# medical-genomics-group/sgVAMP-py

Hardware: AMD Instinct MI355X
Metric: VAMP iterations/sec (and effective LD-matvec GB/s) at M markers, K cohorts (higher is better)
Workload: dtype f64

## Files before the change

sgvamp-py_amd/csrc/common.h:

```cpp
#pragma once
#include <hip/hip_runtime.h>
#include <cstdint>

namespace sgv {

constexpr int WAVE = 64;
constexpr int VTHREADS = 256;
constexpr int CHUNK = 1024;
constexpr int PADV = 128;
constexpr int MAXC = 16;
constexpr int MAXK = 32;
constexpr int MAXCOH = 1024;
constexpr int MAXKG = 8;
constexpr int MAXL = 8;

typedef double d2 __attribute__((ext_vector_type(2)));

#define SGV_GLOBAL __attribute__((address_space(1)))
template <class T>
__device__ __forceinline__ T ldg(const T* p) {
  return *(const SGV_GLOBAL T*)p;
}
template <class T>
__device__ __forceinline__ T ldg_nt(const T* p) {
// ... 234 lines not shown
        if (pa.dot[c]) acc = pre.dot[b] * o;
      }
      const double sm = wave_sum(acc);
      if (lane == 0) s_w[wid][c] = sm;
    }
    __syncthreads();
  }
  if (threadIdx.x < NC)
    partials[(int64_t)pn.part * NC + t] = ((s_w[0][t] + s_w[1][t]) + s_w[2][t]) + s_w[3][t];
}

const char* ab_env(const char* name);

hipError_t launch_read_probe(const double* buf, size_t bytes, double* out, hipStream_t st);

hipError_t launch_coupling(int nc, const CouplingTask* d_tasks, int ntasks, const PassArgs& pa,
                           const double* halo, int64_t hstride, double* cpbuf, int ncp_slots,
                           hipStream_t st);
hipError_t launch_halo_pack(const PassArgs& pa, int nc, int64_t src0, int len0, int64_t src1,
                            int len1, int64_t hstride, double* send, hipStream_t st);
hipError_t launch_ld_pass(int nc, const BlkDesc* d_blks, const RowGroup* d_rg, int nrg,
                          const PassArgs& pa, double* d_partials, hipStream_t st);
int ld_pass_rows_per_group();
hipError_t launch_sym_pass(int nc, int cls, const SymItem* d_items, int nitems,
                           const PassArgs& pa, double* rowpart, double* colpart, hipStream_t st);
hipError_t launch_pk(const PassArgs& pa, int nc, int64_t mpad, double* d_pk, hipStream_t st,
                     bool paired = false);
bool strip_pk_paired(int nc);
hipError_t launch_sym_mfma(int nc, const SymStrip* d_strips, int nstrips, const SymItem* d_sitems,
                           const PassArgs& pa, const double* d_pk, double* rowpart,
                           double* colpart, bool ragged, int pair, int bits, hipStream_t st);
hipError_t launch_sym_mfma_wide(int nc, const SymStrip* d_strips, int nstrips,
                                const SymItem* d_sitems, const PassArgs& pa, const double* d_pk,
                                double* rowpart, double* colpart, bool idle_exit, hipStream_t st);
hipError_t launch_sym_finalize_wide(int nc, const SymPanelW* d_panels, int npanels,
                                    const PassArgs& pa, const double* rowpart,
                                    const double* colpart, double* partials, hipStream_t st);
hipError_t launch_band_walk(int nc, const SymWalk* d_walks, int nwalks, const SymPanel* d_panels,
                            const SymItem* d_items, const double* d_pk, int64_t pk_rows,
                            const PassArgs& pa, double* headbuf, double* carrybuf,
                            const WalkFin* d_fins, int nfins,
                            double* partials, int bits, hipStream_t st);
hipError_t launch_sym_finalize_strip(int nc, const SymPanel* d_panels, int npanels,
                                     const PassArgs& pa, const double* rowpart,
                                     const double* colpart, double* partials, bool ragged,
                                     hipStream_t st);
hipError_t launch_sym_finalize(int nc, int cls, const SymPanel* d_panels, int npanels,
                               const PassArgs& pa, const double* rowpart, const double* colpart,
                               double* partials, hipStream_t st);

hipError_t launch_reduce_blocks(const double* d_part, int nv, const int* d_begin, int nblk,
                                double* d_bsum, hipStream_t st, int op = 0, int ostride = 0,
                                int ooff = 0);
hipError_t launch_reduce_local(const double* d_part, int nv, const int* d_begin, int nblk,
                               const Map16& map, double* d_dst, hipStream_t st, int op = 0);
hipError_t launch_reduce_total(const double* d_bsum_all, int nranks, int nbmax, int nv,
                               const int* d_counts, const Map16& map, double* d_dst,
                               hipStream_t st, int op = 0);

struct DenoiseArgs {
  const double* r1[MAXK];
  double* xhat1;
  double ag[MAXK];
  double a[MAXK], gam1[MAXK];
  double sum_ag;
  double lam;
  int K, nslab;
// ... 245 lines not shown
```

sgvamp-py_amd/csrc/ldplan.hip:

```cpp
#include "ctx.h"

void free_plan(LdPlan& p){
  if (p.d_rg) (void)hipFree(p.d_rg);
  if (p.d_pbeg) (void)hipFree(p.d_pbeg);
  for (int k = 0; k < 4; ++k) {
    if (p.d_items[k]) (void)hipFree(p.d_items[k]);
    if (p.d_panels[k]) (void)hipFree(p.d_panels[k]);
  }
  for (StripSet* q : {&p.s512, &p.wide, &p.rest}) {
    if (q->d_strips) (void)hipFree(q->d_strips);
    if (q->d_sitems) (void)hipFree(q->d_sitems);
    if (q->d_panels) (void)hipFree(q->d_panels);
    if (q->d_wpanels) (void)hipFree(q->d_wpanels);
  }
  if (p.d_ctasks) (void)hipFree(p.d_ctasks);
  if (p.d_walks) (void)hipFree(p.d_walks);
  if (p.d_wpanels) (void)hipFree(p.d_wpanels);
  if (p.d_witems) (void)hipFree(p.d_witems);
  if (p.d_wfins) (void)hipFree(p.d_wfins);
  p = LdPlan();
}

void free_block(LdBlock& lb){
  if (lb.ptr) (void)hipFree(lb.ptr);
// ... 249 lines not shown
  out->ngrp = ngrp;
  out->nstrips = (int)strips.size();
  out->nsitems = (int)sitems.size();
  out->npanels = (int)sp.size();
  out->ragged = false;
  for (const SymStrip& st : strips)
    for (int i = 0; i < st.npan; ++i) out->ragged |= sitems[st.it0 + i].nc < st.ncmax;
  out->pair = (wide || out->ragged) ? 0 : mfma_pair_choice(strips, sitems);
  CHK(upload_table(c, strips, &out->d_strips));
  CHK(upload_table(c, sitems, &out->d_sitems));
  if (wide) {
    CHK(upload_table(c, sp, &out->d_wpanels));
  } else {
    std::vector<SymPanel> p512(sp.size());
    for (size_t i = 0; i < sp.size(); ++i) {
      p512[i] = sp[i].p;
      p512[i].own_sb = sp[i].sb[0];
      p512[i].own_se = sp[i].se[0];
      p512[i].oth_sb = sp[i].sb[1];
      p512[i].oth_se = sp[i].se[1];
    }
    CHK(upload_table(c, p512, &out->d_panels));
  }
  return SGV_OK;
}

static bool wide_pass(int nc) {
  if (nc < 3 || nc > 8) return false;
  const char* e = ab_env("SGV_MF_WIDE");
  if (e && (e[0] == '0' || e[0] == '1')) return e[0] == '1';
  const char* p = ab_env("SGV_MF_PAIR");
  if (p && (p[0] == '0' || p[0] == '1')) return false;
  return true;
}

constexpr int WALK_F32_MIN_NC = 3;
static bool f32_walk_on() {
  const char* e = ab_env("SGV_F32_WALK");
  return e && e[0] == '1';
}
static int band_walk_max_nc() {
  const char* e = ab_env("SGV_BAND_WALK");
  return (e && e[0] == '0') ? 0 : 8;
}

static int plan_walks(sgv_ctx* c, int ld, const std::vector<SymItem>& items,
                      const std::vector<SymPanel>& panels, LdPlan* pl) {
  if (band_walk_max_nc() == 0) return SGV_OK;
  bool any = false;
  for (int b = 0; b < c->nblk; ++b) {
    const LdBlock& lb = c->ldb[ld][b];
    if (lb.fmt != 1) continue;
    if (lb.ext <= 0 || lb.ext > (int64_t)WALK_RMAX * SYM_H) return SGV_OK;
    if (c->bn[b] + SYM_H >= ((int64_t)1 << 31) / (8 * 8)) return SGV_OK;
    any = true;
  }
  if (!any) return SGV_OK;
  if (pl->bits == 32)
    for (const SymItem& it : items)
      if (((uintptr_t)it.P + sizeof(float) * (size_t)(it.c0 - it.r0)) % 16 != 0 || it.w % 4 != 0)
        return fail(c, SGV_ERR_STATE,
                    "walk plan: f32 item (r0 %d, c0 %d, row stride %lld) is not 16-byte aligned",
                    it.r0, it.c0, (long long)it.w);
  std::vector<SymWalk> walks;
  std::vector<WalkFin> fins;
  int hs = 0, cs = 0, bp0 = 0;
// ... 306 lines not shown
    e0 = c->evpool.back();
    c->evpool.pop_back();
    e1 = c->evpool.back();
    c->evpool.pop_back();
  }
  HIPCHK(hipEventRecord(e0, c->st));
  if (pl.halo || pl.nctasks) CHK(coupling_pass(c, pl, nc, pa));
  if (pl.nrg) HIPCHK(launch_ld_pass(nc, c->d_blks[ld], pl.d_rg, pl.nrg, pa, c->d_part, c->st));
  if (pl.npanels) {
    const bool f32 = pl.bits == 32;
    const bool mf = f32 || (c->mfma_min > 0 && nc >= c->mfma_min);
    const int cls = mf ? 1 : sym_class(nc);
    if (mf) {
      const bool walk = pl.nwalks && nc <= band_walk_max_nc() &&
                        (!f32 || (nc >= WALK_F32_MIN_NC && f32_walk_on()));
      double mf_aux = 0.0;
      HIPCHK(launch_pk(pa, nc, c->Mpad, c->d_pk, c->st,
                       walk ? nc > 4 : strip_pk_paired(nc)));
      if (walk) {
        HIPCHK(launch_band_walk(nc, pl.d_walks, pl.nwalks, pl.d_wpanels, pl.d_witems, c->d_pk,
                                c->Mpad, pa,
                                c->d_whead, c->d_wcarry, pl.d_wfins, pl.nwfins, c->d_part, pl.bits,
                                c->st));
      } else {
        const bool usew = !f32 && pl.wide.nstrips > 0 && wide_pass(nc);
        bool side = false;
        auto run_set = [&](const StripSet& ss, bool wide, double* rp, double* cp) -> int {
          for (int g = 0; g < ss.ngrp; ++g) {
            const int s0 = ss.gs[g], ns = ss.gs[g + 1] - s0;
            const int p0 = ss.gp[g], npn = ss.gp[g + 1] - p0;
            const bool split = ss.ngrp > 1;
            if (wide)
              HIPCHK(launch_sym_mfma_wide(nc, ss.d_strips + s0, ns, ss.d_sitems, pa, c->d_pk, rp,
                                          cp, pl.wide_idle, c->st));
            else
              HIPCHK(launch_sym_mfma(nc, ss.d_strips + s0, ns, ss.d_sitems, pa, c->d_pk, rp, cp,
                                     ss.ragged, f32 ? 0 : ss.pair, pl.bits, c->st));
            hipStream_t fs = c->st;
            if (split) {
              HIPCHK(hipEventRecord(c->ev_grp[g % MAXGRP], c->st));
              HIPCHK(hipStreamWaitEvent(c->st_fin, c->ev_grp[g % MAXGRP], 0));
              fs = c->st_fin;
              side = true;
            }
            if (wide)
              HIPCHK(launch_sym_finalize_wide(nc, ss.d_wpanels + p0, npn, pa, rp, cp, c->d_part,
                                              fs));
            else
              HIPCHK(launch_sym_finalize_strip(nc, ss.d_panels + p0, npn, pa, rp, cp, c->d_part,
                                               ss.ragged, fs));
          }
          return SGV_OK;
        };
        if (usew) {
          CHK(run_set(pl.wide, true, c->d_rowpart, c->d_colpart));
          if (pl.rest.nstrips)
            CHK(run_set(pl.rest, false, c->d_rowpart + (size_t)pl.wide.nslots_items * SYM_H * nc,
                        c->d_colpart + (size_t)pl.wide.nstrips * MFW_CW * nc));
          mf_aux = 2.0 * 8.0 * nc * ((double)pl.wide.nsitems * SYM_H +
                                     (double)pl.wide.nstrips * MFW_CW +
                                     (double)pl.rest.nsitems * SYM_H +
                                     (double)pl.rest.nstrips * 512);
        } else {
          CHK(run_set(pl.s512, false, c->d_rowpart, c->d_colpart));
          mf_aux = 2.0 * 8.0 * nc * ((double)pl.s512.nsitems * SYM_H +
                                     (double)pl.s512.nstrips * 512);
        }
// ... 288 lines not shown
```

sgvamp-py_amd/csrc/strip_wave.h:

```cpp
#pragma once
#include "common.h"

#include <type_traits>

namespace sgv {

__device__ __forceinline__ double mfma4(double a, double b, double c) {
  return __builtin_amdgcn_mfma_f64_4x4x4f64(a, b, c, 0, 0, 0);
}

__device__ __forceinline__ void lds_order() {
  __builtin_amdgcn_fence(__ATOMIC_ACQ_REL, "wavefront");
  __builtin_amdgcn_wave_barrier();
}

template <int ORDER>
__device__ __forceinline__ void lds_wait_ge(int* ctr, int v) {
  while (__hip_atomic_load(ctr, ORDER, __HIP_MEMORY_SCOPE_WORKGROUP) < v)
    __builtin_amdgcn_s_sleep(1);
}

typedef float f2 __attribute__((ext_vector_type(2)));
template <class T>
struct Frag;
// ... 118 lines not shown
                                                  bool more, const SymItem& nx,
                                                  uint64_t nxb) const {
    const bool same = g + 1 < ng;
    NextGroup n;
    n.b = same ? curb : nxb;
    n.w = same ? cur.w : (more ? nx.w : 0);
    n.H = same ? cur.H : (more ? nx.H : 1);
    n.nc = same ? cur.nc : nx.nc;
    n.g = same ? g + 1 : 0;
    n.r0 = same ? cur.r0 : nx.r0;
    n.z = col_zero(n.r0);
    return n;
  }

  __device__ __forceinline__ void band_zero(int nci, int t, d2* cf) const {
    const int xc = cw0 + frag_col<LF>(t, lo);
#pragma unroll
    for (int a = 0; a < 4; ++a) {
      cf[a].x = xc < nci ? cf[a].x : 0.0;
      cf[a].y = xc + 1 < nci ? cf[a].y : 0.0;
    }
  }

  __device__ __forceinline__ void tile_exchange(double* sb, const d2* cf, d2* rf) const {
    lds_order();
#pragma unroll
    for (int a = 0; a < 4; ++a)
      *(d2*)(sb + 32 * (4 * (SWZ ? a ^ (bq & 2) : a) + hi) + 2 * (lo ^ hi)) = cf[a];
    lds_order();
#pragma unroll
    for (int r = 0; r < 4; ++r) rf[r] = *(const d2*)(sb + 32 * (4 * r + n4) + 2 * (pc ^ n4));
  }

  __device__ __forceinline__ void reduce_blocks(const double (&drow)[4][NG], double* wb) const {
#pragma unroll
    for (int r = 0; r < 4; ++r)
#pragma unroll
      for (int q = 0; q < NG; ++q) {
        double v = drow[r][q];
        v = v + row_ror<12>(v);
        v = v + row_ror<8>(v);
        if (bq == 0) wb[(4 * r + hi) * RW + 4 * q + n4] = v;
      }
  }

  template <int NT, int CW>
  __device__ __forceinline__ void store_colpart(double* out, int p, int ncol,
                                                const double (&dcol)[NT][2][NG]) const {
#pragma unroll
    for (int q = 0; q < NG; ++q)
      if (4 * q + n4 < ncol) {
#pragma unroll
        for (int t = 0; t < NT; ++t)
          *(d2*)(out + 4 * q * CW + frag_col<LF>(t, p)) = d2{dcol[t][0][q], dcol[t][1][q]};
      }
  }
};

template <class SW, int PD, int NT>
struct FragRing {
  static_assert(PD >= 1 && PD <= NT && NT % PD == 0, "prefetch depth divides the steps");
  static_assert(!SW::W4 || (PD == 2 && NT % 2 == 0), "LF = 2: two super-steps");
  static constexpr int RD = SW::W4 ? NT / 2 : PD;
  typename SW::RV q[RD][4];
  d2 w[SW::W4 ? 2 : 1][4];

// ... 124 lines not shown
```

sgvamp-py_amd/csrc/sym_mfma.hip:

```cpp
#include "strip_wave.h"

namespace sgv {

#ifdef SGV_MF_TRACE
constexpr int MF_TRACE_MAX = 1 << 16;
__device__ unsigned long long g_mf_trace[3 * MF_TRACE_MAX];
#define MF_TRACE_BEGIN const unsigned long long tr_t0 = wall_clock64();
#define MF_TRACE_END                                                          \
  __syncthreads();                                                            \
  if (threadIdx.x == 0 && blockIdx.x < MF_TRACE_MAX) {                        \
    g_mf_trace[3 * blockIdx.x] = tr_t0;                                       \
    g_mf_trace[3 * blockIdx.x + 1] = wall_clock64();                          \
    g_mf_trace[3 * blockIdx.x + 2] = (unsigned long long)__smid();            \
  }
#else
#define MF_TRACE_BEGIN
#define MF_TRACE_END
#endif

constexpr int F32_FORM_DEFAULT = 2;

constexpr int MF_CW = 512;
constexpr int MF_LDP = 34;

template <int NG, int PD, bool RAG = false, bool DEF = false, bool PP = false, class T = double,
          int LF = 1>
__global__ __launch_bounds__(256, 2) void k_sym_mfma(const SymStrip* __restrict__ strips,
                                                     const SymItem* __restrict__ sitems,
                                                     const double* __restrict__ pk, int ncol,
                                                     double* __restrict__ rowpart,
                                                     double* __restrict__ colpart,
                                                     const int* __restrict__ run, int pks) {
  constexpr int NW = 4;
// ... 5 lines not shown
  __shared__ __attribute__((aligned(16))) double stg[NW][16 * 32];
  const SymStrip sp = strips[blockIdx.x];
  if (run && !ldg(run)) return;
  MF_TRACE_BEGIN
  const int lane = threadIdx.x & (WAVE - 1);
  const int wid = __builtin_amdgcn_readfirstlane(threadIdx.x / WAVE);
  SymItem cur = sitems[sp.it0];
  const int cw0 = wid * WC;
  const SW sw(lane, pk + (int64_t)cur.voff * pks, pks, cur.c0, sp.ncmax, cw0, cw0 < SYM_H);
  const int nta = min(NT, sw.steps_to(sw.ncc));
  double* sb = stg[wid];
  double brow[NT][2][NG];
  sw.load_brow(brow);
  double dcol[NT][2][NG];
  zero(dcol);

  uint64_t curb = SW::pbase(cur);
  FragRing<SW, PD, NT> ring;
  double bcn[SW::NB][NG];
  ring.prime(sw, curb, cur);
  sw.load_bcol(cur.r0, cur.H, sw.col_zero(cur.r0), 0, bcn);

#pragma unroll 1
  for (int s = 0; s < sp.npan; ++s) {
    const bool more = s + 1 < sp.npan;
    const SymItem nx = sitems[sp.it0 + (more ? s + 1 : s)];
    const uint64_t nxb = more ? SW::pbase(nx) : (uint64_t)sw.pkb;
    const int ng = (cur.H + 15) / 16;
#pragma unroll 1
    for (int g = 0; g < ng; ++g) {
      const NextGroup nxt = sw.next_group(g, ng, cur, curb, more, nx, nxb);
      double bcol[4][NG];
      sw.hand_bcol(bcn, bcol);
      double drow[4][NG];
      zero(drow);
      const bool colz = sw.col_zero(cur.r0);
      const int ntp = RAG ? min(nta, sw.steps_to(cur.nc)) : nta;
      d2 rfb[DEF ? 2 : 1][4];
#pragma unroll
      for (int t = 0; t < NT; ++t) {
        d2 cf[4];
        d2* rf = rfb[DEF ? (t & 1) : 0];
        ring.step(sw, t, g, curb, cur, nxt, bcn, cf);
        if (t >= ntp) continue;
        if (RAG && cur.nc < sw.ncc) sw.band_zero(cur.nc, t, cf);
        sw.tile_exchange(sb, cf, rf);
        __builtin_amdgcn_s_setprio(1);
        if constexpr (DEF)
          mfma_step_deferred<NG, NT>(t, t == NT - 1 || t + 1 == ntp, colz, cf, rf,
                                     rfb[(t + 1) & 1], bcol, brow, dcol[t], drow);
        else
          mfma_step<NG>(colz, cf, rf, true, bcol, brow[t], dcol[t], drow);
        __builtin_amdgcn_s_setprio(0);
      }
      sw.reduce_blocks(drow, rowbuf + (wid * SYM_H + 16 * g) * RW);
    }
    __syncthreads();
    panel_rows_out<NW, NW * 64, RW>(rowbuf, cur.H, ncol, rowpart + (int64_t)cur.item * SYM_H * ncol);
    __syncthreads();
    cur = nx;
    curb = nxb;
  }
  sw.template store_colpart<NT, MF_CW>(colpart + ((int64_t)sp.slot * ncol + sw.n4) * MF_CW + cw0,
                                       sw.pc, ncol, dcol);
  MF_TRACE_END
}
// ... 22 lines not shown
  const int seg = wid & 3;
  const int h = wid >> 2;
  SymItem cur = sitems[sp.it0];
  const int cw0 = seg * 128 + h * WC;
  const SW sw(lane, pk + (int64_t)cur.voff * pks, pks, cur.c0, sp.ncmax, cw0, seg * 128 < SYM_H);
  const int nta_seg = min(4, max(0, (sw.ncc - seg * 128 + 31) / 32));
  const int nta = min(NT, max(0, nta_seg - NT * h));
  double* sb = stg[wid];
  double brow[NT][2][NG];
  sw.load_brow(brow);
  double dcol[NT][2][NG];
  zero(dcol);

  uint64_t curb = SW::pbase(cur);
  FragRing<SW, PD, NT> ring;
  double bcn[SW::NB][NG];
  ring.prime(sw, curb, cur);
  sw.load_bcol(cur.r0, cur.H, sw.col_zero(cur.r0), 0, bcn);
  if (threadIdx.x < 4) hready[threadIdx.x] = hdone[threadIdx.x] = 0;
  __syncthreads();

  int gg = 0;
#pragma unroll 1
  for (int s = 0; s < sp.npan; ++s) {
    const bool more = s + 1 < sp.npan;
    const SymItem nx = sitems[sp.it0 + (more ? s + 1 : s)];
    const uint64_t nxb = more ? SW::pbase(nx) : (uint64_t)sw.pkb;
    const int ng = (cur.H + 15) / 16;
#pragma unroll 1
    for (int g = 0; g < ng; ++g, ++gg) {
      const NextGroup nxt = sw.next_group(g, ng, cur, curb, more, nx, nxb);
      double bcol[4][NG];
      sw.hand_bcol(bcn, bcol);
      double drow[4][NG];
      zero(drow);
      const bool colz = sw.col_zero(cur.r0);
      d2 rfs[NT][4];
#pragma unroll
      for (int t = 0; t < NT; ++t) {
        d2 cf[4];
        ring.step(sw, t, g, curb, cur, nxt, bcn, cf);
        if (t >= nta) continue;
        sw.tile_exchange(sb, cf, rfs[t]);
        __builtin_amdgcn_s_setprio(1);
        mfma_step<NG>(colz, cf, rfs[t], h == 0, bcol, brow[t], dcol[t], drow);
        __builtin_amdgcn_s_setprio(0);
      }
      double* hs = &hand[gg % HS][seg][0][0];
      if (h == 0) {
        lds_wait_ge<__ATOMIC_ACQUIRE>(&hdone[seg], gg - HS + 1);
#pragma unroll
        for (int r = 0; r < 4; ++r)
#pragma unroll
          for (int q = 0; q < NG; ++q) hs[(r * NG + q) * WAVE + lane] = drow[r][q];
        __hip_atomic_store(&hready[seg], gg + 1, __ATOMIC_RELEASE, __HIP_MEMORY_SCOPE_WORKGROUP);
      }
      if (h == 1) {
        lds_wait_ge<__ATOMIC_ACQUIRE>(&hready[seg], gg + 1);
#pragma unroll
        for (int r = 0; r < 4; ++r)
#pragma unroll
          for (int q = 0; q < NG; ++q) drow[r][q] = hs[(r * NG + q) * WAVE + lane];
        __hip_atomic_store(&hdone[seg], gg + 1, __ATOMIC_RELEASE, __HIP_MEMORY_SCOPE_WORKGROUP);
        __builtin_amdgcn_s_setprio(1);
#pragma unroll
        for (int t = 0; t < NT; ++t)
// ... 37 lines not shown
  const int cw0 = wid * WC;
  const SW sw(lane, pk + (int64_t)cur.voff * PKS, PKS, cur.c0, sp.ncmax, cw0, cw0 < SYM_H);
  const int nta = min(NT, sw.steps_to(sw.ncc));
  const int nact = idle ? min(NW, (sw.ncc + WC - 1) / WC) : NW;
  if (threadIdx.x < MFW_RD) hready[threadIdx.x] = hdone[threadIdx.x] = 0;
  __syncthreads();
  if (wid >= nact) return;
  double* sb = stg[wid];
  double brow[NT][2][NG];
  sw.load_brow(brow);
  double dcol[NT][2][NG];
  zero(dcol);

  uint64_t curb = SW::pbase(cur);
  FragRing<SW, PD, NT> ring;
  double bcn[SW::NB][NG];
  ring.prime(sw, curb, cur);
  sw.load_bcol(cur.r0, cur.H, sw.col_zero(cur.r0), 0, bcn);

  double* outp = colpart + ((int64_t)sp.slot * ncol + sw.n4) * MFW_CW + cw0 + 2 * sw.pc;
  asm volatile("" : "+v"(outp));
  int gg = 0;
#pragma unroll 1
  for (int s = 0; s < sp.npan; ++s) {
    const bool more = s + 1 < sp.npan;
    const SymItem nx = sitems[sp.it0 + (more ? s + 1 : s)];
    const uint64_t nxb = more ? SW::pbase(nx) : (uint64_t)sw.pkb;
    const int ng = (cur.H + 15) / 16;
#pragma unroll 1
    for (int g = 0; g < ng; ++g) {
      const NextGroup nxt = sw.next_group(g, ng, cur, curb, more, nx, nxb);
      double bcol[4][NG];
      sw.hand_bcol(bcn, bcol);
      double drow[4][NG];
      zero(drow);
      const bool colz = sw.col_zero(cur.r0);
      d2 rfb[2][4];
#pragma unroll
      for (int t = 0; t < NT; ++t) {
        d2 cf[4];
        ring.step(sw, t, g, curb, cur, nxt, bcn, cf);
        if (t >= nta) continue;
        sw.tile_exchange(sb, cf, rfb[t & 1]);
        __builtin_amdgcn_s_setprio(1);
        mfma_step_deferred<NG, NT>(t, t == NT - 1 || t + 1 == nta, colz, cf, rfb[t & 1],
                                   rfb[(t + 1) & 1], bcol, brow, dcol[t], drow);
        __builtin_amdgcn_s_setprio(0);
      }
      const int hs = gg % MFW_RD, gen = gg / MFW_RD;
      lds_wait_ge<__ATOMIC_RELAXED>(&hdone[hs], gen);
      sw.reduce_blocks(drow, hand[hs][wid]);
      __builtin_amdgcn_fence(__ATOMIC_RELEASE, "wavefront");
      if (lane == 0)
        __hip_atomic_fetch_add(&hready[hs], 1, __ATOMIC_RELAXED, __HIP_MEMORY_SCOPE_WORKGROUP);
      if (wid == ((g & (NW - 1)) < nact ? (g & (NW - 1)) : 0)) {
        lds_wait_ge<__ATOMIC_RELAXED>(&hready[hs], nact * (gen + 1));
        __builtin_amdgcn_fence(__ATOMIC_ACQUIRE, "wavefront");
        double* dst = rowpart + ((int64_t)cur.item * SYM_H + 16 * g) * ncol;
#pragma unroll
        for (int k = 0; k < (16 * RW + WAVE - 1) / WAVE; ++k) {
          const int e = lane + WAVE * k;
          if (e < 16 * RW) {
            const int row = e / RW, cc = e - row * RW;
            const double* rr = &hand[hs][0][0] + e;
            double v = rr[0];
#pragma unroll
            for (int w = 1; w < NW; ++w) {
              const double x = rr[w * 16 * RW];
              v += w < nact ? x : 0.0;
            }
            if (16 * g + row < cur.H && cc < ncol) dst[row * ncol + cc] = v;
          }
        }
        __builtin_amdgcn_fence(__ATOMIC_RELEASE, "wavefront");
        if (lane == 0)
          __hip_atomic_store(&hdone[hs], gen + 1, __ATOMIC_RELAXED, __HIP_MEMORY_SCOPE_WORKGROUP);
      }
      ++gg;
    }
    cur = nx;
    curb = nxb;
  }
  sw.template store_colpart<NT, MFW_CW>(outp, 0, ncol, dcol);
}

typedef double d4 __attribute__((ext_vector_type(4)));
#define MFMA16(a, b, c) __builtin_amdgcn_mfma_f64_16x16x4f64((a), (b), (c), 0, 0, 0)
template <int PD, bool RAG = false, int TB = 0, class T = double, int LF = 1>
__global__ __launch_bounds__(256, 2) void k_sym_mfma16(const SymStrip* __restrict__ strips,
                                                     const SymItem* __restrict__ sitems,
                                                     const double* __restrict__ pk, int ncol,
                                                     double* __restrict__ rowpart,
                                                     double* __restrict__ colpart,
                                                     const int* __restrict__ run) {
  constexpr int LDP = MF_LDP;
  constexpr int MF_WC = MF_CW / 4;
  constexpr int MF_NT = MF_WC / 32;
  constexpr bool W4 = LF == 2;
  static_assert(!W4 || (sizeof(T) == 4 && PD == 2 && MF_NT % 2 == 0), "LF = 2: float, two super-steps");
  typedef typename std::conditional<W4, f4, typename Frag<T>::raw>::type RV;
  constexpr int RD = W4 ? MF_NT / 2 : PD;
  __shared__ double red[2][4][256];
  __shared__ __attribute__((aligned(16))) double stg[4][16 * LDP];
  constexpr bool BL = TB > 0;
  __shared__ __attribute__((aligned(16))) double bls[BL ? 4 : 1][BL ? TB * 4 : 1][WAVE][2];
  const SymStrip sp = strips[blockIdx.x];
  if (run && !ldg(run)) return;
  const int lane = threadIdx.x & (WAVE - 1);
  const int wid = __builtin_amdgcn_readfirstlane(threadIdx.x / WAVE);
  const int lo = lane & 15, hi = lane >> 4;
  SymItem cur = sitems[sp.it0];
  const int c0 = cur.c0, ncc = sp.ncmax;
  const double* pkb = pk + (int64_t)cur.voff * 16;
  const int cw0 = wid * MF_WC;
  const bool dhalf = cw0 < SYM_H;
  const int nta = W4 ? min(MF_NT, max(0, steps_upto<LF>(ncc - cw0)))
// ... 362 lines not shown
    hipLaunchKernelGGL(k_pack<16>, pg, dim3(256), 0, st, pa, nc, mpad, d_pk);
  return hipGetLastError();
}

hipError_t launch_sym_mfma(int nc, const SymStrip* d_strips, int nstrips, const SymItem* d_sitems,
                           const PassArgs& pa, const double* d_pk, double* rowpart,
                           double* colpart, bool ragged, int pair, int bits, hipStream_t st) {
  if (nc < 1 || nc > 16) return hipErrorInvalidValue;
  if (bits != 64 && bits != 32) return hipErrorInvalidValue;
  const bool f32 = bits == 32;
  if (f32 && pair) return hipErrorInvalidValue;
  if (nstrips <= 0) return hipSuccess;
  const int pks = nc > 8 ? 16 : nc <= 4 ? 4 : 8;
  switch ((nc + 3) / 4) {
    case 1: launch_mf<1>(d_strips, nstrips, d_sitems, d_pk, nc, rowpart, colpart, pa.run, pks, ragged, pair, f32, st); break;
    case 2:
      launch_mf<2, true>(d_strips, nstrips, d_sitems, d_pk, nc, rowpart, colpart, pa.run, pks,
                         ragged, pair, f32, st);
      break;
    default:
      with_strip_inst(f32, ragged, [&](auto i) {
        typedef decltype(i) I;
        hipLaunchKernelGGL((k_sym_mfma16<2, I::rag, I::rag ? 2 : 1, typename I::elem, I::lf>),
                           dim3(nstrips), dim3(256), 0, st, d_strips, d_sitems, d_pk, nc, rowpart,
                           colpart, pa.run);
      });
      break;
  }
  return hipGetLastError();
}

hipError_t launch_sym_mfma_wide(int nc, const SymStrip* d_strips, int nstrips,
                                const SymItem* d_sitems, const PassArgs& pa, const double* d_pk,
                                double* rowpart, double* colpart, bool idle_exit, hipStream_t st) {
  if (nc < 3 || nc > 8) return hipErrorInvalidValue;
  if (nstrips <= 0) return hipSuccess;
  if (nc <= 4)
    hipLaunchKernelGGL((k_sym_mfma_wide<1, 2>), dim3(nstrips), dim3(512), 0, st, d_strips,
                       d_sitems, d_pk, nc, rowpart, colpart, pa.run, idle_exit ? 1 : 0);
  else
    hipLaunchKernelGGL((k_sym_mfma_wide<2, 2, true>), dim3(nstrips), dim3(512), 0, st, d_strips,
                       d_sitems, d_pk, nc, rowpart, colpart, pa.run, idle_exit ? 1 : 0);
  return hipGetLastError();
}

hipError_t launch_sym_finalize_wide(int nc, const SymPanelW* d_panels, int npanels,
                                    const PassArgs& pa, const double* rowpart,
                                    const double* colpart, double* partials, hipStream_t st) {
  if (npanels <= 0) return hipSuccess;
#define FINW_CASE(N)                                                                         \
  case N:                                                                                    \
    hipLaunchKernelGGL(k_sym_finalize_wide<N>, dim3(npanels), dim3(256 * FIN_Q), 0, st,      \
                       d_panels, pa, rowpart, colpart, partials);                            \
    break;
  switch (nc) {
    FINW_CASE(3) FINW_CASE(4) FINW_CASE(5) FINW_CASE(6) FINW_CASE(7) FINW_CASE(8)
    default: return hipErrorInvalidValue;
  }
#undef FINW_CASE
  return hipGetLastError();
}

#ifdef SGV_MF_TRACE
extern "C" int sgv_diag_mf_trace(unsigned long long* out, int n) {
  if (n > MF_TRACE_MAX) n = MF_TRACE_MAX;
  return hipMemcpyFromSymbol(out, HIP_SYMBOL(g_mf_trace), sizeof(unsigned long long) * 3 * n) ==
                 hipSuccess ? n : -1;
}
#endif

static int fin_form(bool ragged, int nc) {
  const char* e = ab_env("SGV_FIN_FORM");
  const int v = (e && (e[0] == '1' || e[0] == '4')) ? e[0] - '0' : 0;
  return v ? v : (ragged && nc <= 8) ? 1 : 4;
}
// ... 28 lines not shown
```

Before: 29.40.

## Add warp-specialized LDS ring loader for the wide symmetric MFMA pass

Adds a new wide symmetric-LD kernel variant in which one or more dedicated loader waves stream LD panel tiles from global memory straight into an LDS ring buffer, using global_load_lds DMA with nontemporal hints. The compute waves consume slots through ready/done flags in LDS instead of issuing their own global loads, so fetching and MFMA work can overlap. The loader variant is picked by an env-tunable code, and for more than four cohorts it defaults to one loader wave, lag 3 and ring depth 6. The existing wide kernels also now prefetch the next group's column operand early. This adds a producer/consumer protocol, more LDS use and one occupancy slot per CU, which risks stalls or synchronisation overhead.

```diff
diff --git a/sgvamp-py_amd/csrc/common.h b/sgvamp-py_amd/csrc/common.h
--- a/sgvamp-py_amd/csrc/common.h
+++ b/sgvamp-py_amd/csrc/common.h
@@ -290,7 +290,8 @@
                            double* colpart, bool ragged, int pair, int bits, hipStream_t st);
 hipError_t launch_sym_mfma_wide(int nc, const SymStrip* d_strips, int nstrips,
                                 const SymItem* d_sitems, const PassArgs& pa, const double* d_pk,
-                                double* rowpart, double* colpart, bool idle_exit, hipStream_t st);
+                                double* rowpart, double* colpart, bool idle_exit, int loader,
+                                hipStream_t st);
 hipError_t launch_sym_finalize_wide(int nc, const SymPanelW* d_panels, int npanels,
                                     const PassArgs& pa, const double* rowpart,
                                     const double* colpart, double* partials, hipStream_t st);
diff --git a/sgvamp-py_amd/csrc/ldplan.hip b/sgvamp-py_amd/csrc/ldplan.hip
--- a/sgvamp-py_amd/csrc/ldplan.hip
+++ b/sgvamp-py_amd/csrc/ldplan.hip
@@ -305,6 +305,15 @@
   const char* p = ab_env("SGV_MF_PAIR");
   if (p && (p[0] == '0' || p[0] == '1')) return false;
   return true;
+}
+
+static int wide_loader(int nc) {
+  constexpr int LOADER_DEFAULT = 136;
+  const char* e = ab_env("SGV_MF_LOADER");
+  if (e && e[0] == '0') return 0;
+  if (e && e[0] && e[1] && e[2]) return std::atoi(e);
+  if (e && e[0] == '1') return LOADER_DEFAULT;
+  return nc > 4 ? LOADER_DEFAULT : 0;
 }
 
 constexpr int WALK_F32_MIN_NC = 3;
@@ -677,7 +686,7 @@
             const bool split = ss.ngrp > 1;
             if (wide)
               HIPCHK(launch_sym_mfma_wide(nc, ss.d_strips + s0, ns, ss.d_sitems, pa, c->d_pk, rp,
-                                          cp, pl.wide_idle, c->st));
+                                          cp, pl.wide_idle, wide_loader(nc), c->st));
             else
               HIPCHK(launch_sym_mfma(nc, ss.d_strips + s0, ns, ss.d_sitems, pa, c->d_pk, rp, cp,
                                      ss.ragged, f32 ? 0 : ss.pair, pl.bits, c->st));
diff --git a/sgvamp-py_amd/csrc/strip_ring.h b/sgvamp-py_amd/csrc/strip_ring.h
--- /dev/null
+++ b/sgvamp-py_amd/csrc/strip_ring.h
@@ -0,0 +1,80 @@
+#pragma once
+
+#if defined(__HIPCC__) || defined(__CUDACC__)
+#define SGV_RING_HD __host__ __device__ __forceinline__
+#else
+#define SGV_RING_HD inline
+#endif
+
+namespace sgv {
+
+constexpr int RING_NW = 8;
+constexpr int RING_HW = 4;
+constexpr int RING_WC = 128;
+constexpr int RING_NT = 4;
+constexpr int RING_SUB = 4096;
+constexpr int RING_PIECE = 1024;
+constexpr int RING_SLOT = RING_HW * RING_SUB;
+constexpr int RING_LAGMAX = 3;
+
+SGV_RING_HD constexpr bool ring_fits(int D, int NL, int LAG) {
+  return NL >= 1 && LAG >= 1 && LAG <= RING_LAGMAX && D > NL * LAG + 2;
+}
+
+SGV_RING_HD int ring_nta(int ncc, int w) {
+  const int n = (ncc - RING_WC * w + 31) / 32;
+  return n < 0 ? 0 : n > RING_NT ? RING_NT : n;
+}
+SGV_RING_HD int ring_nact(int ncc, int idle) {
+  const int n = (ncc + RING_WC - 1) / RING_WC;
+  return idle ? (n < RING_NW ? n : RING_NW) : RING_NW;
+}
+SGV_RING_HD int ring_nfg(int ncc) { return ring_nta(ncc, 0) + ring_nta(ncc, RING_HW); }
+SGV_RING_HD int ring_nwh(int ncc, int t, int h) {
+  int n = 0;
+  for (int w = RING_HW * h; w < RING_HW * h + RING_HW; ++w) n += ring_nta(ncc, w) > t ? 1 : 0;
+  return n;
+}
+SGV_RING_HD int ring_fill_q(int ncc, int t, int h) {
+  const int n4 = ring_nta(ncc, RING_HW);
+  return t + (t < n4 ? t : n4) + h;
+}
+SGV_RING_HD void ring_fill_th(int ncc, int q, int* t, int* h) {
+  const int n4 = ring_nta(ncc, RING_HW);
+  if (q < 2 * n4) {
+    *t = q >> 1;
+    *h = q & 1;
+  } else {
+    *t = q - n4;
+    *h = 0;
+  }
+}
+SGV_RING_HD int ring_slot(int f, int D) { return f % D; }
+SGV_RING_HD int ring_gen(int f, int D) { return f / D; }
+SGV_RING_HD int ring_owner(int f, int NL) { return f % NL; }
+SGV_RING_HD int ring_groups(int H) { return (H + 15) / 16; }
+struct RingWalk {
+  int s, g, ng, q;
+};
+template <class GF>
+SGV_RING_HD bool ring_walk(RingWalk& w, int nfg, int npan, GF groups_of) {
+  while (w.q >= nfg && w.s < npan) {
+    w.q -= nfg;
+    if (++w.g == w.ng) {
+      w.g = 0;
+      if (++w.s < npan) w.ng = groups_of(w.s);
+    }
+  }
+  return w.s < npan;
+}
+SGV_RING_HD int ring_prev_q(int q, int nfg, int D) {
+  const int p = q - D % nfg;
+  return p < 0 ? p + nfg : p;
+}
+SGV_RING_HD int ring_dmas(int nw) { return 4 * nw; }
+SGV_RING_HD int ring_sub_off(int w) { return (w & (RING_HW - 1)) * RING_SUB; }
+
+SGV_RING_HD int ring_src_row(int k, int lane) { return 4 * k + (lane >> 4); }
+SGV_RING_HD int ring_src_pair(int lane) { return (lane & 15) ^ (lane >> 4); }
+
+}
diff --git a/sgvamp-py_amd/csrc/strip_wave.h b/sgvamp-py_amd/csrc/strip_wave.h
--- a/sgvamp-py_amd/csrc/strip_wave.h
+++ b/sgvamp-py_amd/csrc/strip_wave.h
@@ -174,6 +174,16 @@
     for (int r = 0; r < 4; ++r) rf[r] = *(const d2*)(sb + 32 * (4 * r + n4) + 2 * (pc ^ n4));
   }
 
+  __device__ __forceinline__ void slot_read_col(const double* sb, d2* cf) const {
+#pragma unroll
+    for (int a = 0; a < 4; ++a)
+      cf[a] = *(const d2*)(sb + 32 * (4 * (SWZ ? a ^ (bq & 2) : a) + hi) + 2 * (lo ^ hi));
+  }
+  __device__ __forceinline__ void slot_read_row(const double* sb, d2* rf) const {
+#pragma unroll
+    for (int r = 0; r < 4; ++r) rf[r] = *(const d2*)(sb + 32 * (4 * r + n4) + 2 * (pc ^ n4));
+  }
+
   __device__ __forceinline__ void reduce_blocks(const double (&drow)[4][NG], double* wb) const {
 #pragma unroll
     for (int r = 0; r < 4; ++r)
diff --git a/sgvamp-py_amd/csrc/sym_mfma.hip b/sgvamp-py_amd/csrc/sym_mfma.hip
--- a/sgvamp-py_amd/csrc/sym_mfma.hip
+++ b/sgvamp-py_amd/csrc/sym_mfma.hip
@@ -1,4 +1,5 @@
 #include "strip_wave.h"
+#include "strip_ring.h"
 
 namespace sgv {
 
@@ -70,6 +71,7 @@
       const NextGroup nxt = sw.next_group(g, ng, cur, curb, more, nx, nxb);
       double bcol[4][NG];
       sw.hand_bcol(bcn, bcol);
+      sw.load_bcol(nxt.r0, nxt.H, nxt.z, nxt.g, bcn);
       double drow[4][NG];
       zero(drow);
       const bool colz = sw.col_zero(cur.r0);
@@ -158,6 +160,7 @@
       const NextGroup nxt = sw.next_group(g, ng, cur, curb, more, nx, nxb);
       double bcol[4][NG];
       sw.hand_bcol(bcn, bcol);
+      sw.load_bcol(nxt.r0, nxt.H, nxt.z, nxt.g, bcn);
       double drow[4][NG];
       zero(drow);
       const bool colz = sw.col_zero(cur.r0);
@@ -261,6 +264,7 @@
       const NextGroup nxt = sw.next_group(g, ng, cur, curb, more, nx, nxb);
       double bcol[4][NG];
       sw.hand_bcol(bcn, bcol);
+      sw.load_bcol(nxt.r0, nxt.H, nxt.z, nxt.g, bcn);
       double drow[4][NG];
       zero(drow);
       const bool colz = sw.col_zero(cur.r0);
@@ -311,6 +315,270 @@
     curb = nxb;
   }
   sw.template store_colpart<NT, MFW_CW>(outp, 0, ncol, dcol);
+}
+
+__device__ __forceinline__ void glds16_nt(const void* gsrc, unsigned lds_dst) {
+  unsigned keep;
+  asm volatile(
+      "s_mov_b32 %0, m0\n\ts_mov_b32 m0, %2\n\ts_nop 0\n\t"
+      "global_load_lds_dwordx4 %1, off nt\n\ts_mov_b32 m0, %0"
+      : "=&s"(keep)
+      : "v"(gsrc), "s"(lds_dst)
+      : "memory");
+}
+__device__ __forceinline__ void vm_wait_dma4(int n) {
+  switch (n) {
+    case 0: asm volatile("s_waitcnt vmcnt(0)" ::: "memory"); break;
+    case 1: asm volatile("s_waitcnt vmcnt(4)" ::: "memory"); break;
+    case 2: asm volatile("s_waitcnt vmcnt(8)" ::: "memory"); break;
+    case 3: asm volatile("s_waitcnt vmcnt(12)" ::: "memory"); break;
+    case 4: asm volatile("s_waitcnt vmcnt(16)" ::: "memory"); break;
+    case 5: asm volatile("s_waitcnt vmcnt(20)" ::: "memory"); break;
+    case 6: asm volatile("s_waitcnt vmcnt(24)" ::: "memory"); break;
+    case 7: asm volatile("s_waitcnt vmcnt(28)" ::: "memory"); break;
+    case 8: asm volatile("s_waitcnt vmcnt(32)" ::: "memory"); break;
+    case 9: asm volatile("s_waitcnt vmcnt(36)" ::: "memory"); break;
+    case 10: asm volatile("s_waitcnt vmcnt(40)" ::: "memory"); break;
+    case 11: asm volatile("s_waitcnt vmcnt(44)" ::: "memory"); break;
+    default: asm volatile("s_waitcnt vmcnt(48)" ::: "memory"); break;
+  }
+}
+
+template <int NL, int LAG, int D>
+__device__ __forceinline__ void ring_loader(const SymStrip& sp, const SymItem* __restrict__ sitems,
+                                            int j, int lane, unsigned ring_lds, int* sready,
+                                            int* sdone) {
+  const int ncc = sp.ncmax;
+  const int nfg = ring_nfg(ncc);
+  const int xc0 = 2 * ring_src_pair(lane);
+  __builtin_amdgcn_s_setprio(3);
+  SymItem cur = sitems[sp.it0];
+  RingWalk wk = {0, 0, ring_groups(cur.H), j};
+  int pslot[LAG], pgen[LAG], pcnt[LAG];
+#pragma unroll
+  for (int i = 0; i < LAG; ++i) pslot[i] = -1, pgen[i] = 0, pcnt[i] = 0;
+#pragma unroll 1
+  for (int f = j;; f += NL, wk.q += NL) {
+    const int s0 = wk.s;
+    if (!ring_walk(wk, nfg, sp.npan, [&](int s) { return ring_groups(sitems[sp.it0 + s].H); })) break;
+    if (wk.s != s0) cur = sitems[sp.it0 + wk.s];
+    const int g = wk.g, q = wk.q;
+    const int slot = ring_slot(f, D), gen = ring_gen(f, D);
+    int t, h;
+    ring_fill_th(ncc, q, &t, &h);
+    const int nw = ring_nwh(ncc, t, h);
+    if (gen > 0) {
+      int tp, hp;
+      ring_fill_th(ncc, ring_prev_q(q, nfg, D), &tp, &hp);
+      lds_wait_ge<__ATOMIC_RELAXED>(&sdone[slot], ring_nwh(ncc, tp, hp));
+      __builtin_amdgcn_fence(__ATOMIC_ACQUIRE, "wavefront");
+      if (lane == 0)
+        __hip_atomic_store(&sdone[slot], 0, __ATOMIC_RELAXED, __HIP_MEMORY_SCOPE_WORKGROUP);
+    }
+    const double* pb = (const double*)cur.P + (cur.c0 - cur.r0);
+    const double* rowp[4];
+#pragma unroll
+    for (int k = 0; k < 4; ++k) {
+      const int rB = 16 * g + ring_src_row(k, lane);
+      rowp[k] = pb + (int64_t)(rB < cur.H ? rB : cur.H - 1) * cur.w;
+    }
+    const unsigned dst = ring_lds + slot * RING_SLOT;
+#pragma unroll 1
+    for (int w = RING_HW * h; w < RING_HW * h + nw; ++w) {
+      const int xc = RING_WC * w + 32 * t + xc0;
+      const int col = xc < ncc ? xc : 0;
+#pragma unroll
+      for (int k = 0; k < 4; ++k)
+        glds16_nt(rowp[k] + col,
+                  __builtin_amdgcn_readfirstlane(dst + ring_sub_off(w) + k * RING_PIECE));
+    }
+    int later = nw;
+#pragma unroll
+    for (int i = 1; i < LAG; ++i) later += pcnt[i];
+    if (pslot[0] >= 0) {
+      vm_wait_dma4(later);
+      if (lane == 0)
+        __hip_atomic_store(&sready[pslot[0]], pgen[0] + 1, __ATOMIC_RELAXED,
+                           __HIP_MEMORY_SCOPE_WORKGROUP);
+    }
+#pragma unroll
+    for (int i = 0; i + 1 < LAG; ++i) pslot[i] = pslot[i + 1], pgen[i] = pgen[i + 1], pcnt[i] = pcnt[i + 1];
+    pslot[LAG - 1] = slot, pgen[LAG - 1] = gen, pcnt[LAG - 1] = nw;
+  }
+  vm_wait_dma4(0);
+#pragma unroll
+  for (int i = 0; i < LAG; ++i)
+    if (pslot[i] >= 0 && lane == 0)
+      __hip_atomic_store(&sready[pslot[i]], pgen[i] + 1, __ATOMIC_RELAXED,
+                         __HIP_MEMORY_SCOPE_WORKGROUP);
+}
+
+template <int NG, int NL, int LAG, int D, int TB = 0, bool PP = false>
+__global__ __launch_bounds__(512 + 64 * NL, 1) void k_sym_mfma_wide_ld(
+    const SymStrip* __restrict__ strips, const SymItem* __restrict__ sitems,
+    const double* __restrict__ pk, int ncol, double* __restrict__ rowpart,
+    double* __restrict__ colpart, const int* __restrict__ run, int idle) {
+  constexpr int NW = RING_NW;
+  constexpr int WC = RING_WC;
+  constexpr int NT = RING_NT;
+  static_assert(WC * NW == MFW_CW && ring_fits(D, NL, LAG), "ring shape");
+  typedef StripWave<NG, PP> SW;
+  constexpr int RW = SW::RW;
+  __shared__ __attribute__((aligned(1024))) double ring[D * RING_SLOT / 8];
+  __shared__ __attribute__((aligned(16))) double hand[MFW_RD][NW][16 * RW];
+  __shared__ int hready[MFW_RD], hdone[MFW_RD];
+  __shared__ int sready[D], sdone[D];
+  static_assert(TB == 0 || TB == 1, "at most the last step's operands in LDS");
+  constexpr int NR = NT - TB;
+  __shared__ __attribute__((aligned(16))) double bls[TB ? NW : 1][2][WAVE][NG];
+  const SymStrip sp = strips[blockIdx.x];
+  if (run && !ldg(run)) return;
+  const int lane = threadIdx.x & (WAVE - 1);
+  const int wid = __builtin_amdgcn_readfirstlane(threadIdx.x / WAVE);
+  if (threadIdx.x < MFW_RD) hready[threadIdx.x] = hdone[threadIdx.x] = 0;
+  if (threadIdx.x < D) sready[threadIdx.x] = sdone[threadIdx.x] = 0;
+  __syncthreads();
+  if (wid >= NW) {
+    ring_loader<NL, LAG, D>(sp, sitems, wid - NW, lane,
+                            (unsigned)(uintptr_t)(__attribute__((address_space(3))) void*)ring,
+                            sready, sdone);
+    return;
+  }
+  SymItem cur = sitems[sp.it0];
+  constexpr int PKS = 4 * NG;
+  const int cw0 = wid * WC;
+  const SW sw(lane, pk + (int64_t)cur.voff * PKS, PKS, cur.c0, sp.ncmax, cw0, cw0 < SYM_H);
+  const int nta = ring_nta(sw.ncc, wid);
+  const int nfg = ring_nfg(sw.ncc);
+  const int nact = ring_nact(sw.ncc, idle);
+  if (wid >= nact) return;
+  const double* sub = ring + ring_sub_off(wid) / 8;
+  double brow[NR][2][NG];
+  {
+    double b[NT][2][NG];
+    sw.load_brow(b);
+#pragma unroll
+    for (int e = 0; e < 2; ++e)
+#pragma unroll
+      for (int q = 0; q < NG; ++q) {
+#pragma unroll
+        for (int t = 0; t < NR; ++t) brow[t][e][q] = b[t][e][q];
+        if constexpr (TB) bls[wid][e][lane][q] = b[NT - 1][e][q];
+      }
+    lds_order();
+  }
+  double dcol[NT][2][NG];
+  zero(dcol);
+  double bcn[SW::NB][NG];
+  sw.load_bcol(cur.r0, cur.H, sw.col_zero(cur.r0), 0, bcn);
+
+  auto release = [&](int slot) {
+    __builtin_amdgcn_fence(__ATOMIC_RELEASE, "wavefront");
+    if (lane == 0)
+      __hip_atomic_fetch_add(&sdone[slot], 1, __ATOMIC_RELAXED, __HIP_MEMORY_SCOPE_WORKGROUP);
+  };
+  int gg = 0;
+#pragma unroll 1
+  for (int s = 0; s < sp.npan; ++s) {
+    const bool more = s + 1 < sp.npan;
+    const SymItem nx = sitems[sp.it0 + (more ? s + 1 : s)];
+    const int ng = (cur.H + 15) / 16;
+#pragma unroll 1
+    for (int g = 0; g < ng; ++g) {
+      const NextGroup nxt = sw.next_group(g, ng, cur, 0, more, nx, 0);
+      double bcol[4][NG];
+      sw.hand_bcol(bcn, bcol);
+      sw.load_bcol(nxt.r0, nxt.H, nxt.z, nxt.g, bcn);
+      double drow[4][NG];
+      zero(drow);
+      const bool colz = sw.col_zero(cur.r0);
+      int pslot = 0;
+#pragma unroll
+      for (int t = 0; t < NT; ++t) {
+        if (t >= nta) continue;
+        const bool last = t == NT - 1 || t + 1 == nta;
+        d2 cf[4], rp[4], rf[4];
+        const int f = gg * nfg + ring_fill_q(sw.ncc, t, wid / RING_HW);
+        const int slot = ring_slot(f, D);
+        lds_wait_ge<__ATOMIC_RELAXED>(&sready[slot], ring_gen(f, D) + 1);
+        __builtin_amdgcn_fence(__ATOMIC_ACQUIRE, "wavefront");
+        sw.slot_read_col(sub + slot * (RING_SLOT / 8), cf);
+        if (t > 0) {
+          sw.slot_read_row(sub + pslot * (RING_SLOT / 8), rp);
+          release(pslot);
+        }
+        __builtin_amdgcn_s_setprio(1);
+#pragma unroll
+        for (int a = 0; a < 4; ++a) {
+          if (!colz) col_mfma<NG>(cf[a], bcol[a], dcol[t]);
+          if (t > 0) {
+#pragma unroll
+            for (int r = 2 * (a & 1); r < 2 * (a & 1) + 2; ++r)
+#pragma unroll
+              for (int q = 0; q < NG; ++q)
+                drow[r][q] = mfma4(a < 2 ? rp[r].x : rp[r].y, brow[t > 0 ? t - 1 : 0][a < 2 ? 0 : 1][q],
+                                   drow[r][q]);
+          }
+          if (a == 1 && last) {
+            __builtin_amdgcn_sched_barrier(0);
+            sw.slot_read_row(sub + slot * (RING_SLOT / 8), rf);
+            release(slot);
+          }
+        }
+        if (last) {
+          if constexpr (TB) {
+            if (t == NT - 1) {
+              double bl[2][NG];
+#pragma unroll
+              for (int e = 0; e < 2; ++e)
+#pragma unroll
+                for (int q = 0; q < NG; ++q) bl[e][q] = bls[wid][e][lane][q];
+              row_mfma<NG>(rf, bl, drow);
+            } else {
+              row_mfma<NG>(rf, brow[t < NR ? t : 0], drow);
+            }
+          } else {
+            row_mfma<NG>(rf, brow[t < NR ? t : 0], drow);
+          }
+        }
+        __builtin_amdgcn_s_setprio(0);
+        pslot = slot;
+      }
+      const int hs = gg % MFW_RD, gen = gg / MFW_RD;
+      lds_wait_ge<__ATOMIC_RELAXED>(&hdone[hs], gen);
+      sw.reduce_blocks(drow, hand[hs][wid]);
+      __builtin_amdgcn_fence(__ATOMIC_RELEASE, "wavefront");
+      if (lane == 0)
+        __hip_atomic_fetch_add(&hready[hs], 1, __ATOMIC_RELAXED, __HIP_MEMORY_SCOPE_WORKGROUP);
+      if (wid == ((g & (NW - 1)) < nact ? (g & (NW - 1)) : 0)) {
+        lds_wait_ge<__ATOMIC_RELAXED>(&hready[hs], nact * (gen + 1));
+        __builtin_amdgcn_fence(__ATOMIC_ACQUIRE, "wavefront");
+        double* dst = rowpart + ((int64_t)cur.item * SYM_H + 16 * g) * ncol;
+#pragma unroll
+        for (int k = 0; k < (16 * RW + WAVE - 1) / WAVE; ++k) {
+          const int e = lane + WAVE * k;
+          if (e < 16 * RW) {
+            const int row = e / RW, cc = e - row * RW;
+            const double* rr = &hand[hs][0][0] + e;
+            double v = rr[0];
+#pragma unroll
+            for (int w = 1; w < NW; ++w) {
+              const double x = rr[w * 16 * RW];
+              v += w < nact ? x : 0.0;
+            }
+            if (16 * g + row < cur.H && cc < ncol) dst[row * ncol + cc] = v;
+          }
+        }
+        __builtin_amdgcn_fence(__ATOMIC_RELEASE, "wavefront");
+        if (lane == 0)
+          __hip_atomic_store(&hdone[hs], gen + 1, __ATOMIC_RELAXED, __HIP_MEMORY_SCOPE_WORKGROUP);
+      }
+      ++gg;
+    }
+    cur = nx;
+  }
+  sw.template store_colpart<NT, MFW_CW>(colpart + ((int64_t)sp.slot * ncol + sw.n4) * MFW_CW + cw0,
+                                        sw.pc, ncol, dcol);
 }
 
 typedef double d4 __attribute__((ext_vector_type(4)));
@@ -739,15 +1007,34 @@
 
 hipError_t launch_sym_mfma_wide(int nc, const SymStrip* d_strips, int nstrips,
                                 const SymItem* d_sitems, const PassArgs& pa, const double* d_pk,
-                                double* rowpart, double* colpart, bool idle_exit, hipStream_t st) {
+                                double* rowpart, double* colpart, bool idle_exit, int loader,
+                                hipStream_t st) {
   if (nc < 3 || nc > 8) return hipErrorInvalidValue;
   if (nstrips <= 0) return hipSuccess;
-  if (nc <= 4)
-    hipLaunchKernelGGL((k_sym_mfma_wide<1, 2>), dim3(nstrips), dim3(512), 0, st, d_strips,
-                       d_sitems, d_pk, nc, rowpart, colpart, pa.run, idle_exit ? 1 : 0);
-  else
-    hipLaunchKernelGGL((k_sym_mfma_wide<2, 2, true>), dim3(nstrips), dim3(512), 0, st, d_strips,
-                       d_sitems, d_pk, nc, rowpart, colpart, pa.run, idle_exit ? 1 : 0);
+#define WIDE_LD(NL, LAG, D)                                                                   \
+  case 100 * NL + 10 * LAG + D:                                                               \
+    if (nc <= 4)                                                                              \
+      hipLaunchKernelGGL((k_sym_mfma_wide_ld<1, NL, LAG, D, 0>), dim3(nstrips),                  \
+                         dim3(512 + 64 * NL), 0, st, d_strips, d_sitems, d_pk, nc, rowpart,   \
+                         colpart, pa.run, idle_exit ? 1 : 0);                                 \
+    else                                                                                      \
+      hipLaunchKernelGGL((k_sym_mfma_wide_ld<2, NL, LAG, D, 1, true>), dim3(nstrips),            \
+                         dim3(512 + 64 * NL), 0, st, d_strips, d_sitems, d_pk, nc, rowpart,   \
+                         colpart, pa.run, idle_exit ? 1 : 0);                                 \
+    break;
+  switch (loader) {
+    case 0:
+      if (nc <= 4)
+        hipLaunchKernelGGL((k_sym_mfma_wide<1, 2>), dim3(nstrips), dim3(512), 0, st, d_strips,
+                           d_sitems, d_pk, nc, rowpart, colpart, pa.run, idle_exit ? 1 : 0);
+      else
+        hipLaunchKernelGGL((k_sym_mfma_wide<2, 2, true>), dim3(nstrips), dim3(512), 0, st, d_strips,
+                           d_sitems, d_pk, nc, rowpart, colpart, pa.run, idle_exit ? 1 : 0);
+      break;
+    WIDE_LD(1, 3, 6) WIDE_LD(1, 2, 6) WIDE_LD(2, 1, 6) WIDE_LD(1, 1, 4)
+    default: return hipErrorInvalidValue;
+  }
+#undef WIDE_LD
   return hipGetLastError();
 }
 
```

Result: slower. 19.73 (-32.9%).
